# domerin0/rnn-speech

Measured on AMD Instinct MI355X. Metric: audio_frames_per_sec_train_3x512_lstm_ctc, higher is better.
Workload: dtype f32

## Files before the change

### include/amdspeech.h

```cpp
#ifndef AMDSPEECH_H
#define AMDSPEECH_H

#include <stddef.h>
#include <stdint.h>

#ifdef __cplusplus
extern "C" {
#endif

#define AMDSPEECH_OK 0
#define AMDSPEECH_EINVAL (-1)
#define AMDSPEECH_EHIP (-2)
#define AMDSPEECH_EUNSUPPORTED (-3)
#define AMDSPEECH_ETIMEOUT (-4)

int amdspeech_version(void);
const char* amdspeech_last_error(void);
int amdspeech_device_cu_count(void);

int amdspeech_linear_fwd(void* stream, const float* x, const float* w, const float* b,
                         float* y, int M, int K, int N);
int amdspeech_linear_bwd(void* stream, const float* x, const float* w, const float* dy,
                         float* dx, float* dw, float* db, int M, int K, int N);

// ... 107 lines not shown
                           const float* kernels, long kernel_stride, const float* biases, long bias_stride,
                           const int* lengths, const float* h0, const float* c0, const amdspeech_ctc_head* head);
int amdspeech_lstm_bwd_ctc(void* stream, const amdspeech_lstm_desc* d, void* ws,
                           const float* kernels, long kernel_stride, float* dkernels, float* dbiases, long bias_stride,
                           const int* lengths, const amdspeech_ctc_head* head);

int amdspeech_lstm_dropout_multipliers(void* stream, const amdspeech_lstm_desc* d, int which, int layer, float* out);

enum { AMDSPEECH_LSTM_PATH_FLOW = 0, AMDSPEECH_LSTM_PATH_BIG1 = 1, AMDSPEECH_LSTM_PATH_BIG = 2, AMDSPEECH_LSTM_PATH_HOIST = 3,
       AMDSPEECH_LSTM_PATH_DIAG = 4, AMDSPEECH_LSTM_PATH_DIAG_BF3 = 5 };
typedef struct amdspeech_lstm_plan_info {
    int fwd_path, bwd_path, nmt, kb, mv, wpx, uw, fwd_mt, pair, bf16p, bf16p_reserved, xw_parts, nfw, w_pieces, dz0_inkernel, flow2_q;
} amdspeech_lstm_plan_info;
int amdspeech_lstm_plan(const amdspeech_lstm_desc* d, int C, int U, amdspeech_lstm_plan_info* out);
int amdspeech_lstm_plan_xw_halves(const amdspeech_lstm_desc* d, int C, int U);

enum {
    AMDSPEECH_BIDIR_WS_Z0 = 0, AMDSPEECH_BIDIR_WS_YTOP_FW = 1, AMDSPEECH_BIDIR_WS_YTOP_BW = 2, AMDSPEECH_BIDIR_WS_DYTOP_FW = 3,
    AMDSPEECH_BIDIR_WS_DYTOP_BW = 4, AMDSPEECH_BIDIR_WS_DZ0 = 5, AMDSPEECH_BIDIR_WS_HFINAL = 6, AMDSPEECH_BIDIR_WS_CFINAL = 7
};
size_t amdspeech_lstm_bidir_workspace_bytes(const amdspeech_lstm_desc* d);
void* amdspeech_lstm_bidir_ws_ptr(const amdspeech_lstm_desc* d, void* ws, int which);
long amdspeech_lstm_bidir_layer_stride(const amdspeech_lstm_desc* d);
int amdspeech_lstm_bidir_path(const amdspeech_lstm_desc* d);
int amdspeech_lstm_bidir_fwd(void* stream, const amdspeech_lstm_desc* d, void* ws, const float* const* kernels,
                             const float* const* biases, const int* lengths, const float* h0, const float* c0);
int amdspeech_lstm_bidir_bwd(void* stream, const amdspeech_lstm_desc* d, void* ws, const float* const* kernels,
                             float* const* dkernels, float* const* dbiases, const int* lengths);
int amdspeech_lstm_bidir_status(const amdspeech_lstm_desc* d, void* ws);
int amdspeech_lstm_bidir_dropout_multipliers(void* stream, const amdspeech_lstm_desc* d, int dir, int which, int layer, float* out);
// ... 202 lines not shown
```

### rnn-speech_amd/csrc/lstm.hip

```cpp
#include "common.h"
#include "gemm_core.h"
#include "ctc_core.h"
#include <stdlib.h>
#include <string.h>
#include <type_traits>
#include <mutex>
#include <unordered_map>

namespace amdspeech {

#define FLOW_WEIGHTS_RESIDENT() __builtin_amdgcn_s_waitcnt(0x0F70)
static unsigned long long* dev_trace_ptr() {
#ifdef AMDSPEECH_DEVTRACE
    if (const char* e = dev_knob_str("AMDSPEECH_TRACE_PTR")) return reinterpret_cast<unsigned long long*>(strtoull(e, nullptr, 0));
#endif
    return nullptr;
}
#ifndef BIG_WEIGHTS_RESIDENT
#define BIG_WEIGHTS_RESIDENT 1
#endif

struct LstmLayout {
    size_t wp, wq, z, hs, cs, gates, dg, dztop, dz0, dc, xp0, xp, hp, dgp, sync, xph, hph, dxh, prec, pdown, xwp, bigring, wopack, bfs, total;
    size_t fwd_set = 0;
// ... 291 lines not shown
}

static bool use_big_fwd(const amdspeech_lstm_desc* d) {
    static const int env = runtime_switch("AMDSPEECH_BIG", 1);
    return env != 0 && !(d->flags & AMDSPEECH_LSTM_PER_DIAGONAL) && d->precision >= 0 && d->precision <= 2 && d->H == 1024 &&
           (d->B + 15) / 16 <= 4 && device_cus() == 256 &&
           (size_t)2 * ((d->B + 15) / 16 * 16) * d->H * 4 < (1ull << 32);
}

static bool use_flow(const amdspeech_lstm_desc* d) {
    static const int env = runtime_switch("AMDSPEECH_FLOW", 1);
    return env != 0 && !(d->flags & AMDSPEECH_LSTM_PER_DIAGONAL) && flow_shape_ok(d) && device_cus() == 256 && d->L * ((d->B + 15) / 16) <= 8;
}

template <bool CF>
static void (*flow_fwd_kernel(int kb, int pr, int mv, int mh))(FlowArgs) {
    switch (kb) {
        case 1: return lstm_fwd_flow2<1, 0, 0, CF>;
        case 2: return pr == 2 ? lstm_fwd_flow2<2, 2, 0, CF> : (pr == 1 ? lstm_fwd_flow2<2, 1, 0, CF> : lstm_fwd_flow2<2, 0, 0, CF>);
        case 3: return lstm_fwd_flow2<3, 0, 0, CF>;
        default:
            if (pr == 0 && mv == 1) return mh == 1 ? lstm_fwd_flow2<4, 0, 1, CF, 1> : lstm_fwd_flow2<4, 0, 1, CF>;
            return pr == 2 ? lstm_fwd_flow2<4, 2, 0, CF> : (pr == 1 ? lstm_fwd_flow2<4, 1, 0, CF> : lstm_fwd_flow2<4, 0, 0, CF>);
    }
}
template <bool CF>
static void (*flow_bwd_kernel(int kb, int pr))(FlowBwdArgs) {
    if (pr == 2) return kb == 2 ? lstm_bwd_flow2<2, 2, CF> : lstm_bwd_flow2<4, 2, CF>;
    if (pr == 1) return kb == 2 ? lstm_bwd_flow2<2, 1, CF> : lstm_bwd_flow2<4, 1, CF>;
    return kb == 1 ? lstm_bwd_flow2<1, 0, CF> : (kb == 2 ? lstm_bwd_flow2<2, 0, CF> : (kb == 3 ? lstm_bwd_flow2<3, 0, CF> : lstm_bwd_flow2<4, 0, CF>));
}
static int flow_fill_fwd_panels(hipStream_t s, const amdspeech_lstm_desc* d, float* ws, const LstmLayout& lo, int set) {
    const size_t bph = (size_t)(d->B + 15) / 16 * 16 * d->H;
    float* base = ws + (size_t)set * lo.fwd_set;
    AS_CHECK_HIP(hipMemsetD32Async(reinterpret_cast<hipDeviceptr_t>(base + lo.xph + (size_t)d->T * bph), (int)FLOW_SENTINEL,
                                   (size_t)d->L * d->T * bph, s));
    AS_CHECK_HIP(hipMemsetD32Async(reinterpret_cast<hipDeviceptr_t>(base + lo.hph), (int)FLOW_SENTINEL, (size_t)d->L * (d->T + 1) * bph, s));
// ... 140 lines not shown
    int xw_half;
    bool big_ring;
    bool bf16p_reserved;
    bool bf16p;
    Path fwd, bwd;
    bool pair;
    int uw;
    unsigned long long limit;
    void (*fwd_diag)(FwdArgs); int fwd_mt;
    void (*bwd_diag)(BwdArgs);
    void (*fwd_big)(BigFwdArgs); void (*bwd_big)(BigBwdArgs);
    void (*fwd_flow)(FlowArgs); void (*bwd_flow)(FlowBwdArgs);
    size_t fwd_lds, bwd_lds;
    int mv, wpx, wpw;
    int mh;
    int nfw;
    int dz0_inkernel;
    int w_pieces, w_t0, w_dz0;
    bool w_deal;
};

struct FlowGemmShare { int pieces, percent; bool set; };
static FlowGemmShare flow_gemm_share() {
    static const FlowGemmShare g = [] {
        FlowGemmShare r{8, 38, false};
        if (const char* e = dev_knob_str("AMDSPEECH_FLOW_GEMM")) {
            r.set = true;
            r.pieces = atoi(e);
            if (const char* q = strchr(e, ':')) r.percent = atoi(q + 1);
        }
// ... 24 lines not shown
    const Path diag = pr != 0 ? Path::diag_bf3 : Path::diag;
    p.fwd = flow ? Path::flow : big ? (p.pair && big1_env == 2 ? Path::big1 : Path::big) : diag;
    p.bwd = flow ? Path::flow : (p.pair && p.bf16p) ? Path::big1 : big ? Path::big
          : (pr == 0 && H >= 768 && p.nmt >= 2) ? Path::hoist : diag;
    p.uw = (flow || big) ? 16 : pick_uw(d);

    p.fwd_mt = p.nmt % 2 == 0 ? 2 : 1;
    if (pr != 0) p.fwd_diag = lstm_fwd_step_bf3<8>;
    else if (p.uw == 8) p.fwd_diag = p.fwd_mt == 2 ? lstm_fwd_step<8, 8, 8, false, 2> : lstm_fwd_step<8, 8, 8, false, 1>;
    else p.fwd_diag = p.fwd_mt == 2 ? lstm_fwd_step<4, 8, 8, false, 2> : lstm_fwd_step<4, 8, 8, false, 1>;
    p.bwd_diag = pr != 0 ? lstm_bwd_step_bf3<8> : lstm_bwd_step<8, 8, true>;
    p.fwd_big = pr == 2 ? lstm_fwd_big<2> : (pr == 1 ? lstm_fwd_big<1> : lstm_fwd_big<0>);
    p.bwd_big = pr == 2 ? lstm_bwd_big<2> : (pr == 1 ? lstm_bwd_big<1> : lstm_bwd_big<0>);
    if (!flow) return p;

    static const int workers_env = runtime_switch("AMDSPEECH_FLOW_FWD_WORKERS", 2);
    const int groups = L * p.nmt, spare = 8 - groups;
    p.wpw = 8;
    if (workers_env != 0 && p.xw_parts > 0)
        for (int waves = 4; waves <= 8 && p.mv == 0; waves += 4) {
            const int per = fwd_worker_wgs_per_xcd(d, waves);
            if (per <= 32 - FWD2_WORKER_RESERVE) { p.mv = 1; p.wpx = per; p.wpw = waves; }
        }
    p.mh = (workers_env != 1 && p.mv == 1 && p.wpw == 4 && p.xw_half > 0) ? 1 : 0;
    if (head != nullptr) p.nfw = ctc_head_nfw(d, head->C, head->U, p.wpx);
    const int kb = H / 128;
    p.fwd_flow = head != nullptr ? flow_fwd_kernel<true>(kb, pr, p.mv, p.mh) : flow_fwd_kernel<false>(kb, pr, p.mv, p.mh);
    p.bwd_flow = head != nullptr ? flow_bwd_kernel<true>(kb, pr) : flow_bwd_kernel<false>(kb, pr);
    p.fwd_lds = head != nullptr ? (size_t)2 * CF_FOLLOW_TEAM_FLOATS * sizeof(float) : 0;
    p.bwd_lds = ((size_t)2 * 1024 + 2 * 8 * 256 + (FLOW2_WINDOW ? 2 : 1) * 8 * kb * 256 + (size_t)(flow2_q(kb, pr) - 1) * 1024) * sizeof(float);
    const size_t lds_workers = (size_t)2 * 2 * 2 * BK * LDS_LD * sizeof(float);
    if (p.bwd_lds < lds_workers) p.bwd_lds = lds_workers;
    if (p.bwd_lds < (size_t)2 * CF_LEAD_TEAM_FLOATS * sizeof(float)) p.bwd_lds = (size_t)2 * CF_LEAD_TEAM_FLOATS * sizeof(float);

    const FlowGemmShare g = flow_gemm_share();
    const bool workers = g.pieces > 0 && g.percent > 0 && T >= 64 && groups < 8 && H % 128 == 0;
    const int share = g.set ? g.percent : (pr != 0 ? (head != nullptr ? g.percent / 2 - 1 : g.percent * 3 / 4) : g.percent);
    static const int dz0_in = runtime_switch("AMDSPEECH_FLOW_DZ0", 1);
    p.dz0_inkernel = dz0_in ? 1 : 0;
    p.w_dz0 = (p.dz0_inkernel || workers) ? 0 : 1;
    p.w_pieces = workers ? g.pieces : 0;
    static const int deal = runtime_switch("AMDSPEECH_FLOW_WORKER_DEAL", -1);
// ... 761 lines not shown
    const bool flow_bwd = p.bwd == Path::flow;
    static_assert((int)Path::flow == AMDSPEECH_LSTM_PATH_FLOW && (int)Path::big1 == AMDSPEECH_LSTM_PATH_BIG1 &&
                  (int)Path::big == AMDSPEECH_LSTM_PATH_BIG && (int)Path::hoist == AMDSPEECH_LSTM_PATH_HOIST &&
                  (int)Path::diag == AMDSPEECH_LSTM_PATH_DIAG && (int)Path::diag_bf3 == AMDSPEECH_LSTM_PATH_DIAG_BF3, "amdspeech.h");
    *out = amdspeech_lstm_plan_info{(int)p.fwd, (int)p.bwd, p.nmt, p.fwd == Path::flow ? d->H / 128 : 0, p.mv, p.wpx, p.uw, p.fwd_mt,
                                    p.pair ? 1 : 0, p.bf16p ? 1 : 0, p.bf16p_reserved ? 1 : 0, p.xw_parts, p.nfw, p.w_pieces,
                                    p.dz0_inkernel, flow_bwd ? flow2_q(d->H / 128, d->precision) : 0};
    return AMDSPEECH_OK;
}
extern "C" int amdspeech_lstm_plan_xw_halves(const amdspeech_lstm_desc* d, int C, int U) {
    if (check_desc(d) != AMDSPEECH_OK) return -1;
    amdspeech_ctc_head h{};
    h.C = C; h.U = U;
    const LstmPlan p = lstm_plan(d, C > 0 ? &h : nullptr);
    return 2 * p.mv + p.mh;
}
extern "C" int amdspeech_lstm_ctc_fusable(const amdspeech_lstm_desc* d, int C, int U) {
    if (check_desc(d) != AMDSPEECH_OK) return 0;
    amdspeech_ctc_head h{};
    h.C = C; h.U = U;
    return lstm_plan(d, &h).nfw > 0 ? 1 : 0;
}
static int check_head(const amdspeech_ctc_head* h, bool bwd) {
    AS_CHECK_ARG(h != nullptr, "lstm_*_ctc: null head");
    AS_CHECK_ARG(h->w_out && h->b_out && h->logits && h->dense_labels && h->loss && h->ctc_ws && (!bwd || h->dlogits),
                 "lstm_*_ctc: null pointer in the head");
    AS_CHECK_ARG(((uintptr_t)h->w_out % 16) == 0 && ((uintptr_t)h->ctc_ws % 256) == 0, "lstm_*_ctc: W_o must be 16-byte, the CTC workspace 256-byte aligned");
    return AMDSPEECH_OK;
}
extern "C" int amdspeech_lstm_fwd_ctc(void* stream, const amdspeech_lstm_desc* d, void* ws, const float* kernels,
// ... 384 lines not shown
```

### rnn-speech_amd/csrc/lstm_flow_fwd.h

```cpp

#ifndef FWD2_GATHER_AT
#define FWD2_GATHER_AT 1
#endif
#ifndef FWD2_WORKER_LAG
#define FWD2_WORKER_LAG 4
#endif

template <int KB, int MV, int MH, int NTW>
__device__ __forceinline__ void fwd_x_worker(const FlowArgs& a, const int role, const int lane, const unsigned long long t_begin) {
    constexpr int H = 128 * KB, NKBX = H / 16, NU = H / 16, NT = 4;
    constexpr bool HALF = NTW != NT;
    constexpr int J0 = NT - NTW;
    static_assert(NTW == 4 || (NTW == 2 && MH == 1), "x-product workers: full roles, or half roles of a launch that carries them");
    const int T = a.T, nmt = (a.B + 15) / 16;
    int r = __builtin_amdgcn_readfirstlane(role);
    const int part = HALF ? MV : r % MV;
    if (!HALF) r /= MV;
    const int ub = r % NU; r /= NU;
    const int mb = r % nmt;
    const int l = r / nmt;
    if (l >= a.L) return;
    const size_t bph = (size_t)nmt * 16 * H;
    float4 w[8][NTW];
    {
        const float* wp = a.wp + ((size_t)(l * NU + ub) * (2 * NKBX)) * (NT * 256) + lane * 4;
#pragma unroll
        for (int wv = 0; wv < 8; ++wv)
#pragma unroll
            for (int j = 0; j < NTW; ++j) w[wv][j] = *reinterpret_cast<const float4*>(wp + (size_t)((wv * KB + KB - 1 - part) * NT + J0 + j) * 256);
    }
    const float* xsrc = l == 0 ? a.xp0 : a.xph + (size_t)l * T * bph;
    const auto rx = __builtin_amdgcn_make_buffer_rsrc(const_cast<float*>(xsrc), 0, (unsigned)((size_t)T * bph * 4), 0x00020000);
    const size_t fs = (size_t)a.L * nmt * NU * (MV * 1024 + MH * 512);
    const auto ro = __builtin_amdgcn_make_buffer_rsrc(a.xwp, 0, (unsigned)((size_t)T * fs * 4), 0x00020000);
    const unsigned lane_off = (unsigned)((((size_t)mb * NKBX + (KB - 1 - part)) * 256 + lane * 4) * 4);
    const unsigned out_off = HALF ? (unsigned)(((size_t)a.L * nmt * NU * MV * 1024 + (((size_t)l * nmt + mb) * NU + ub) * 512 + lane * 4) * 4)
                                  : (unsigned)((((((size_t)l * nmt + mb) * NU + ub) * MV + part) * 1024 + lane * 4) * 4);
    const unsigned par = a.xw_par & 1u;
    bool dead = false;
    u32x4_f xa[8] = {}, xb[8] = {};
    auto load_l2 = [&](u32x4_f& dst, unsigned vo, unsigned so) { asm volatile("buffer_load_dwordx4 %0, %1, %2, %3 offen" : "+v"(dst) : "v"(vo), "s"(rx), "s"(so)); };
    auto load_mem = [&](u32x4_f& dst, unsigned vo, unsigned so) { asm volatile("buffer_load_dwordx4 %0, %1, %2, %3 offen sc1" : "+v"(dst) : "v"(vo), "s"(rx), "s"(so)); };
    auto issue = [&](auto bottom, u32x4_f (&buf)[8], int t) {
        const unsigned base = (unsigned)((size_t)(t < T ? t : T - 1) * bph * 4);
#pragma unroll
        for (int wv = 0; wv < 8; ++wv) {
            const unsigned vo = lane_off + (unsigned)(wv * KB * 1024);
            if (decltype(bottom)::value) load_l2(buf[wv], vo, base); else load_mem(buf[wv], vo, base);
        }
    };
    FLOW_WEIGHTS_RESIDENT();
    u32x4_f pr = (u32x4_f){0u, 0u, 0u, 0u};
    auto probe = [&](int t) {
        const int tp = t + FWD2_WORKER_LAG < T ? t + FWD2_WORKER_LAG : T - 1;
        load_mem(pr, lane_off, (unsigned)((size_t)tp * bph * 4));
    };
    auto landed12 = [&](u32x4_f (&buf)[8]) {
        asm volatile("s_waitcnt vmcnt(%9)" : "+v"(pr), "+v"(buf[0]), "+v"(buf[1]), "+v"(buf[2]), "+v"(buf[3]), "+v"(buf[4]), "+v"(buf[5]), "+v"(buf[6]), "+v"(buf[7]) : "n"(8 + NTW));
    };
    auto landed0 = [&](u32x4_f (&buf)[8]) {
        asm volatile("s_waitcnt vmcnt(0)" : "+v"(pr), "+v"(buf[0]), "+v"(buf[1]), "+v"(buf[2]), "+v"(buf[3]), "+v"(buf[4]), "+v"(buf[5]), "+v"(buf[6]), "+v"(buf[7]));
    };
    auto pending_any = [&](const u32x4_f (&buf)[8]) -> bool {
        unsigned bad = 0u;
#pragma unroll
        for (int wv = 0; wv < 8; ++wv) bad |= (unsigned)flow_pending(buf[wv]);
        return bad != 0u;
    };
#if defined(AMDSPEECH_DEVTRACE) && AMDSPEECH_DEVTRACE == 5
    const bool wtracing = a.trace != nullptr && l == a.trace_layer && ub == 3 && mb == 0 && part == 0 && lane == 0;
#define FXWSTAMP(i) do { if (wtracing && t >= 500 && t < 508) a.trace[128 + (t - 500) * 8 + (i)] = wall_clock64(); } while (0)
#else
#define FXWSTAMP(i) do { } while (0)
#endif
    auto work = [&](auto bottom, int t, u32x4_f (&buf)[8]) __attribute__((always_inline)) {
        FXWSTAMP(0);
        landed12(buf);
        FXWSTAMP(1);
        if (!decltype(bottom)::value) {
            if (__any(flow_pending(pr) || pending_any(buf)) && !dead) {
                while (true) {
                    if (wall_clock64() - t_begin > a.limit) { dead = true; if (lane == 0) atomicOr(a.err, 8u); break; }
                    __builtin_amdgcn_s_sleep(4);
                    probe(t);
                    issue(bottom, buf, t);
                    landed0(buf);
                    if (!__any(flow_pending(pr) || pending_any(buf))) break;
                }
            }
        }
        FXWSTAMP(2);
        probe(t + 1);
        f32x4 acc[NTW];
#pragma unroll
        for (int j = 0; j < NTW; ++j) acc[j] = (f32x4){0.f, 0.f, 0.f, 0.f};
#pragma unroll
        for (int wv = 0; wv < 8; ++wv)
#pragma unroll
            for (int j = 0; j < NTW; ++j) {
                acc[j] = __builtin_amdgcn_mfma_f32_16x16x4f32(__uint_as_float(buf[wv][0]), w[wv][j].x, acc[j], 0, 0, 0);
                acc[j] = __builtin_amdgcn_mfma_f32_16x16x4f32(__uint_as_float(buf[wv][1]), w[wv][j].y, acc[j], 0, 0, 0);
                acc[j] = __builtin_amdgcn_mfma_f32_16x16x4f32(__uint_as_float(buf[wv][2]), w[wv][j].z, acc[j], 0, 0, 0);
                acc[j] = __builtin_amdgcn_mfma_f32_16x16x4f32(__uint_as_float(buf[wv][3]), w[wv][j].w, acc[j], 0, 0, 0);
            }
        const unsigned fo = out_off + (unsigned)((size_t)t * fs * 4);
#pragma unroll
        for (int i = 0; i < NTW; ++i) {
            f32x4 v;
            if constexpr (HALF) v = (f32x4){acc[0][2 * i], acc[1][2 * i], acc[0][2 * i + 1], acc[1][2 * i + 1]};
            else v = (f32x4){acc[0][i], acc[1][i], acc[2][i], acc[3][i]};
            __builtin_amdgcn_raw_buffer_store_b128(flow_tag(v, par), ro, fo + (unsigned)(i * 1024), 0, 16);
        }
        __builtin_amdgcn_sched_barrier(0);
        FXWSTAMP(3);
        issue(bottom, buf, t + 2);
        FXWSTAMP(4);
    };
#undef FXWSTAMP
    auto run = [&](auto bottom) __attribute__((always_inline)) {
        probe(0);
        if (!decltype(bottom)::value) {
            landed0(xa);
            if (__any(flow_pending(pr)) && !dead) {
                while (true) {
                    if (wall_clock64() - t_begin > a.limit) { dead = true; if (lane == 0) atomicOr(a.err, 8u); break; }
                    __builtin_amdgcn_s_sleep(4);
                    probe(0);
                    landed0(xa);
                    if (!__any(flow_pending(pr))) break;
                }
            }
        }
        issue(bottom, xa, 0);
        landed0(xa);
        issue(bottom, xb, 1);
        for (int t = 0; t < T; t += 2) {
            work(bottom, t, xa);
            if (t + 1 < T) work(bottom, t + 1, xb);
        }
        landed0(xa);
        landed0(xb);
    };
    if (l == 0) run(std::true_type{}); else run(std::false_type{});
}

#define FLOW_G(T, p) ((T __attribute__((address_space(1)))*)(p))
template <typename Args>
__device__ __forceinline__ Args flow_args_again() {
    typedef unsigned args_u4 __attribute__((ext_vector_type(4)));
    typedef const args_u4 __attribute__((address_space(4))) * cptr;
    static_assert(sizeof(Args) % 16 == 0, "argument struct: a whole number of 16-byte pieces");
    unsigned long long p = (unsigned long long)__builtin_amdgcn_kernarg_segment_ptr();
    asm("" : "+s"(p));
    const cptr q = (cptr)p;
    args_u4 buf[sizeof(Args) / 16];
#pragma unroll
    for (unsigned i = 0; i < sizeof(Args) / 16; ++i) buf[i] = q[i];
    Args r;
    __builtin_memcpy(&r, buf, sizeof(Args));
    return r;
}
template <int H>
__device__ __forceinline__ void ctc_follower_call(const CtcFlow& c, int wg, int nwg) {
    extern __shared__ __attribute__((aligned(16))) float cf_lds[];
    if (c.B <= nwg * 2) ctc_follower<H, 1>(c, cf_lds, wg, nwg);
    else ctc_follower<H, 2>(c, cf_lds, wg, nwg);
}

template <int KB, int PR, int MV, bool CF = false, int MH = 0>
__global__ __launch_bounds__(512) void lstm_fwd_flow2(FlowArgs a_in) {
    constexpr bool BF3 = PR != 0;
    static_assert(MV >= 0 && MV < KB && (MV == 0 || PR == 0), "x-product workers: exact f32 only, and one K block of the x half stays");
    static_assert(MH == 0 || (MH == 1 && MV > 0 && KB - MV >= 2), "half roles: beside full roles, and one whole K block of the x half stays");
    constexpr int KX = KB - MV;
    constexpr int NTL = MH ? 2 : 4;
    constexpr int MVA = MV > 0 ? MV : 1;
    constexpr int UW = 16, NT = 4, H = 128 * KB, NKBX = H / 16, NW = 8;
    __shared__ __attribute__((aligned(16))) float red_[1][NW][256][NT];
    __shared__ __attribute__((aligned(16))) float outbox[2][8][256];
    __shared__ unsigned s_ticket;
    const int lane = threadIdx.x & 63, wave = __builtin_amdgcn_readfirstlane(threadIdx.x >> 6);
    unsigned xcc;
    asm volatile("s_getreg_b32 %0, hwreg(HW_REG_XCC_ID)" : "=s"(xcc));
    xcc &= 0xF;
    if (threadIdx.x == 0) s_ticket = atomicAdd(a_in.tickets + xcc, 1u);
    __syncthreads();
    const int grp = (int)xcc, ub = __builtin_amdgcn_readfirstlane((int)s_ticket);
    if (grp >= a_in.L * ((a_in.B + 15) / 16)) {
        const int first = a_in.L * ((a_in.B + 15) / 16);
        if (MV > 0 && ub < a_in.w_wpx && wave < a_in.w_wpw)
            fwd_x_worker<KB, MVA, MH, 4>(a_in, (((grp - first) * a_in.w_wpx + ub) * a_in.w_wpw + wave), lane, wall_clock64());
        else if (MH > 0 && ub < a_in.w_wpx) {
            if constexpr (MH > 0) fwd_x_worker<KB, MVA, MH, 2>(a_in, (((grp - first) * a_in.w_wpx + ub) * 4 + wave - 4), lane, wall_clock64());
        }
        else if (CF && a_in.cf_on && ub >= a_in.w_wpx && ub < a_in.w_wpx + a_in.cf_nfw) {
            if constexpr (CF) ctc_follower_call<H>(a_in.cf, (grp - first) * a_in.cf_nfw + (ub - a_in.w_wpx), (8 - first) * a_in.cf_nfw);
        }
        return;
    }
    const FlowArgs a = CF ? flow_args_again<FlowArgs>() : a_in;
    const int T = a.T, B = a.B;
    const int nmt = (B + 15) / 16;
    if (ub >= H / UW) return;
    const int l = grp / nmt, mb = grp % nmt;
    const size_t bph = (size_t)nmt * 16 * H;
    const unsigned long long t_begin = wall_clock64();
    const unsigned long long c_begin = __builtin_readcyclecounter();

    float4 wx[KX][NT], wh[KB][NT];
    {
        const float __attribute__((address_space(1)))* wp = FLOW_G(const float, a.wp) + ((size_t)(l * (H / UW) + ub) * (2 * NKBX)) * (NT * 256) + lane * 4;
#pragma unroll
        for (int kb = 0; kb < KB; ++kb)
#pragma unroll
            for (int j = 0; j < NT; ++j) {
                if (kb < KX && (kb < KX - 1 || j < NTL)) { const f32x4 v = *(const f32x4 __attribute__((address_space(1)))*)(wp + (size_t)((wave * KB + kb) * NT + j) * 256); wx[kb][j] = make_float4(v[0], v[1], v[2], v[3]); }
                { const f32x4 v = *(const f32x4 __attribute__((address_space(1)))*)(wp + (size_t)((NKBX + wave * KB + kb) * NT + j) * 256); wh[kb][j] = make_float4(v[0], v[1], v[2], v[3]); }
            }
    }
    constexpr int KP = BF3 ? KB / 2 : 1;
    u32x4_f wxh[KP][NT], wxl[KP][NT], whh[KP][NT], whl[KP][NT];
    if constexpr (BF3) {
#pragma unroll
        for (int jb = 0; jb < KB / 2; ++jb)
#pragma unroll
            for (int j = 0; j < NT; ++j) {
                const float xx[8] = {wx[2 * jb][j].x, wx[2 * jb][j].y, wx[2 * jb][j].z, wx[2 * jb][j].w,
                                     wx[2 * jb + 1][j].x, wx[2 * jb + 1][j].y, wx[2 * jb + 1][j].z, wx[2 * jb + 1][j].w};
                flow_bf3_split(xx, wxh[jb][j], wxl[jb][j]);
                const float xh[8] = {wh[2 * jb][j].x, wh[2 * jb][j].y, wh[2 * jb][j].z, wh[2 * jb][j].w,
                                     wh[2 * jb + 1][j].x, wh[2 * jb + 1][j].y, wh[2 * jb + 1][j].z, wh[2 * jb + 1][j].w};
// ... 144 lines not shown
#pragma unroll
        for (int j = 0; j < NJ; ++j) acc[j] = __builtin_amdgcn_mfma_f32_16x16x4f32(__uint_as_float(v[2]), w[j].z, acc[j], 0, 0, 0);
#pragma unroll
        for (int j = 0; j < NJ; ++j) acc[j] = __builtin_amdgcn_mfma_f32_16x16x4f32(__uint_as_float(v[3]), w[j].w, acc[j], 0, 0, 0);
        __builtin_amdgcn_sched_barrier(0);
#else
#pragma unroll
        for (int j = 0; j < NJ; ++j) {
            acc[j] = __builtin_amdgcn_mfma_f32_16x16x4f32(__uint_as_float(v[0]), w[j].x, acc[j], 0, 0, 0);
            acc[j] = __builtin_amdgcn_mfma_f32_16x16x4f32(__uint_as_float(v[1]), w[j].y, acc[j], 0, 0, 0);
            acc[j] = __builtin_amdgcn_mfma_f32_16x16x4f32(__uint_as_float(v[2]), w[j].z, acc[j], 0, 0, 0);
            acc[j] = __builtin_amdgcn_mfma_f32_16x16x4f32(__uint_as_float(v[3]), w[j].w, acc[j], 0, 0, 0);
        }
#endif
    };
    auto half_product = [&](const auto& v, const auto& w, const u32x4_f (&wh_)[KP][NT], const u32x4_f (&wl_)[KP][NT],
                            auto between, auto last_tiles) __attribute__((always_inline)) {
        constexpr int NB = (int)(sizeof(v) / sizeof(v[0]));
        if constexpr (BF3) {
#pragma unroll
            for (int jb = 0; jb < KB / 2; ++jb) {
                between(2 * jb);
                between(2 * jb + 1);
                const float x[8] = {__uint_as_float(v[2 * jb][0]), __uint_as_float(v[2 * jb][1]), __uint_as_float(v[2 * jb][2]),
                                    __uint_as_float(v[2 * jb][3]), __uint_as_float(v[2 * jb + 1][0]), __uint_as_float(v[2 * jb + 1][1]),
                                    __uint_as_float(v[2 * jb + 1][2]), __uint_as_float(v[2 * jb + 1][3])};
                u32x4_f ah, al;
                flow_bf3_split(x, ah, al);
#pragma unroll
                for (int j = 0; j < NT; ++j) acc[j] = flow_bf_mma<PR>(acc[j], ah, al, wh_[jb][j], wl_[jb][j]);
            }
        } else {
#pragma unroll
            for (int kb = 0; kb < NB; ++kb) {
                between(kb);
                if (kb == NB - 1) mma_block(v[kb], w[kb], last_tiles);
                else mma_block(v[kb], w[kb], std::integral_constant<int, NT>{});
            }
        }
    };
    auto fsig = [](float x) __attribute__((always_inline)) { return __builtin_amdgcn_rcpf(1.0f + __builtin_amdgcn_exp2f(-1.4426950408889634f * x)); };
    auto ftanh = [](float x) __attribute__((always_inline)) {
        const float x2 = x * x;
        const float small = x * (1.0f + x2 * (-0.33333334f + x2 * (0.13333334f - 0.053968254f * x2)));
        const float big = 1.0f - 2.0f * __builtin_amdgcn_rcpf(1.0f + __builtin_amdgcn_exp2f(2.8853900817779268f * x));
        return fabsf(x) < 0.25f ? small : big;
    };
    auto stores = [&](int t) __attribute__((always_inline)) {
        const int sl = threadIdx.x - 256;
        const float (&ob)[8][256] = outbox[t & 1];
        const float zv = ob[6][sl] * zmult(a.drop, l + 1, (uint32_t)((size_t)t * B * H + e));
// ... 27 lines not shown
        const float cv = live ? cn : c_prev;
        const float zv = live ? hn : 0.0f;
        __hip_atomic_store(FLOW_G(float, a.hph) + ((size_t)l * (T + 1) + t + 1) * bph + po, hval, __ATOMIC_RELAXED, __HIP_MEMORY_SCOPE_WORKGROUP);
        const int sl = threadIdx.x;
        float (&ob)[8][256] = outbox[t & 1];
        ob[0][sl] = gi; ob[1][sl] = gj; ob[2][sl] = gf; ob[3][sl] = go;
        ob[4][sl] = cv; ob[5][sl] = hval; ob[6][sl] = zv; ob[7][sl] = c_prev;
        c_prev = cv; h_prev = hval;
    };
    auto x_half = [&](auto xpol, int t, u32x4_f (&xnext)[KX], bool gather_h) __attribute__((always_inline)) {
#pragma unroll
        for (int j = 0; j < NT; ++j) acc[j] = (f32x4){0.f, 0.f, 0.f, 0.f};
        if (t + 1 < T) {
            if (decltype(xpol)::value != 2 && !(ASM && FWD2_EARLY_XCHECK)) settle(Remote{}, xnext, rx, (unsigned)((size_t)(t + 1) * bph * 4));
            half_product(xnext, wx, wxh, wxl, [&](int kb) {
                if (gather_h && kb == (FWD2_GATHER_AT < KX ? FWD2_GATHER_AT : KX - 1)) {
                    __builtin_amdgcn_sched_barrier(0);
                    issue(Local{}, hv, rh, (unsigned)((size_t)(t + 1) * bph * 4));
                    __builtin_amdgcn_sched_barrier(0);
                }
            }, std::integral_constant<int, NTL>{});
        }
    };
#ifndef FWD2_ISSUE_AT_TOP
#define FWD2_ISSUE_AT_TOP 0
#endif
    constexpr bool TOP = ASM && FWD2_ISSUE_AT_TOP != 0;
    auto step = [&](auto xpol, int t, u32x4_f (&xnext)[KX], u32x4_f (&xfree)[KX], u32x4_f (&wcur)[MVA], u32x4_f (&wfree)[MVA],
                    u32x2_f& hcur, u32x2_f& hfree) __attribute__((always_inline)) {
        F2STAMP(0);
        if constexpr (TOP) {
// ... 96 lines not shown
```

### rnn-speech_amd/lib.py

```python
import ctypes as C
import os

HERE = os.path.dirname(os.path.abspath(__file__))
LIB_PATH = os.environ.get("AMDSPEECH_LIB") or os.path.join(HERE, "libamdspeech.so")


class AmdSpeechError(RuntimeError):
    pass


class DataflowTimeout(AmdSpeechError):
    """amdspeech_lstm_status returned AMDSPEECH_ETIMEOUT: a whole-sequence launch gave up waiting.  The mini-batch's results are
    invalid; it can be repeated on the launch-per-diagonal kernels.  Any OTHER error of that call is a device fault."""


ETIMEOUT = -4
ECALLBACK = -100


class LstmDesc(C.Structure):
    _fields_ = [("T", C.c_int), ("B", C.c_int), ("H", C.c_int), ("L", C.c_int),
                ("keep_in", C.c_float), ("keep_out", C.c_float), ("seed", C.c_uint64),
                ("precision", C.c_int), ("flags", C.c_int)]

# ... 117 lines not shown
    "amdspeech_lstm_fwd": (_I, [_P, C.POINTER(LstmDesc), _P, _P, _L, _P, _L, _P, _P, _P]),
    "amdspeech_lstm_status": (_I, [C.POINTER(LstmDesc), _P]),
    "amdspeech_lstm_workspace_release": (_I, [_P, _P]),
    "amdspeech_lstm_beside_forward": (_I, [_P, _P]),
    "amdspeech_lstm_beside_tail": (_I, [_P, _P]),
    "amdspeech_lstm_bwd": (_I, [_P, C.POINTER(LstmDesc), _P, _P, _L, _P, _P, _L, _P]),
    "amdspeech_lstm_ctc_fusable": (_I, [C.POINTER(LstmDesc), _I, _I]),
    "amdspeech_lstm_pair_fusable": (_I, [C.POINTER(LstmDesc)]),
    "amdspeech_lstm_fwd_pair": (_I, [_P, C.POINTER(LstmDesc), _P, _P, _P, C.POINTER(LstmDesc), _P, _P, _P, _L, _L, _P, _P, _P]),
    "amdspeech_lstm_bwd_pair": (_I, [_P, C.POINTER(LstmDesc), _P, _P, _P, _P, C.POINTER(LstmDesc), _P, _P, _P, _P, _L, _L, _P]),
    "amdspeech_lstm_fwd_ctc": (_I, [_P, C.POINTER(LstmDesc), _P, _P, _L, _P, _L, _P, _P, _P, C.POINTER(CtcHead)]),
    "amdspeech_lstm_bwd_ctc": (_I, [_P, C.POINTER(LstmDesc), _P, _P, _L, _P, _P, _L, _P, C.POINTER(CtcHead)]),
    "amdspeech_lstm_dropout_multipliers": (_I, [_P, C.POINTER(LstmDesc), _I, _I, _P]),
    "amdspeech_lstm_plan": (_I, [C.POINTER(LstmDesc), _I, _I, C.POINTER(LstmPlanInfo)]),
    "amdspeech_lstm_plan_xw_halves": (_I, [C.POINTER(LstmDesc), _I, _I]),
    "amdspeech_lstm_bidir_workspace_bytes": (_SZ, [C.POINTER(LstmDesc)]),
    "amdspeech_lstm_bidir_ws_ptr": (_P, [C.POINTER(LstmDesc), _P, _I]),
    "amdspeech_lstm_bidir_layer_stride": (_L, [C.POINTER(LstmDesc)]),
    "amdspeech_lstm_bidir_path": (_I, [C.POINTER(LstmDesc)]),
    "amdspeech_lstm_bidir_fwd": (_I, [_P, C.POINTER(LstmDesc), _P, _P, _P, _P, _P, _P]),
    "amdspeech_lstm_bidir_bwd": (_I, [_P, C.POINTER(LstmDesc), _P, _P, _P, _P, _P]),
    "amdspeech_lstm_bidir_status": (_I, [C.POINTER(LstmDesc), _P]),
    "amdspeech_lstm_bidir_dropout_multipliers": (_I, [_P, C.POINTER(LstmDesc), _I, _I, _I, _P]),
    "amdspeech_ctc_workspace_bytes": (_SZ, [_I, _I, _I, _I]),
    "amdspeech_ctc_plan": (_I, [_I, _I, _I, _I, C.POINTER(CtcPlanInfo)]),
    "amdspeech_ctc_loss_fwd_bwd": (_I, [_P, _P, _P, _P, _I, _I, _I, _I, _P, _P, _P]),
    "amdspeech_ctc_loss_fwd_bwd_staged": (_I, [_P, _P, _P, _P, _I, _I, _I, _I, _P, _P, _P, _I]),
    "amdspeech_ctc_align_workspace_bytes": (_SZ, [_I, _I, _I, _I]),
    "amdspeech_ctc_align_plan": (_I, [_I, _I, _I, _I, C.POINTER(CtcPlanInfo)]),
    "amdspeech_ctc_align": (_I, [_P, _P, _P, _P, _I, _I, _I, _I, _P, _P, _P, _P, _P, _P]),
# ... 98 lines not shown
```

### rnn-speech_amd/ops.py

```python
import ctypes as C
import os

import torch

from . import lib as _l

MODE_MFCC, MODE_FBANK = 0, 1


def _stream():
    return C.c_void_p(torch.cuda.current_stream().cuda_stream)


def _p(t):
    return C.c_void_p(t.data_ptr()) if t is not None else C.c_void_p(0)


def _chk_f32(*ts):
    for t in ts:
        if t is None:
            continue
        if not (t.is_cuda and t.dtype == torch.float32 and t.is_contiguous()):
            raise ValueError("expected a contiguous float32 device tensor, got %s %s" % (t.dtype, t.device))

# ... 343 lines not shown
                    _l.LSTM_PER_DIAGONAL if per_diagonal else 0)
    info = _l.LstmPlanInfo()
    _l.check(ws.lib.amdspeech_lstm_plan(C.byref(d), c_u[0], c_u[1], C.byref(info)), "lstm_plan")
    out = _plan_dict(info)
    out["fwd_path"], out["bwd_path"] = _l.LSTM_PATHS[out["fwd_path"]], _l.LSTM_PATHS[out["bwd_path"]]
    return out


def lstm_plan_xw_halves(ws, head=None, per_diagonal=False):
    c_u = (0, 0) if head is None else ((head.c.C, head.c.U) if isinstance(head, CtcHead) else (int(head[0]), int(head[1])))
    d = _l.LstmDesc(ws.desc.T, ws.desc.B, ws.desc.H, ws.desc.L, ws.desc.keep_in, ws.desc.keep_out, ws.desc.seed, ws.desc.precision,
                    _l.LSTM_PER_DIAGONAL if per_diagonal else 0)
    n = int(ws.lib.amdspeech_lstm_plan_xw_halves(C.byref(d), c_u[0], c_u[1]))
    if n < 0:
        raise ValueError("lstm_plan_xw_halves: bad descriptor")
    return n


def lstm_fwd(ws, kernels, kernel_stride, biases, bias_stride, lengths, h0=None, c0=None, training=False, per_diagonal=False, head=None):
    _chk_i32(lengths)
    _chk_f32(h0, c0)
    root, key = ws._root, (ws.T, int(ws.desc.precision))
    if per_diagonal:
        root._armed, training = None, False
    armed = _ARM and root._armed is not None and root._armed["fwd"] == key
    root._armed = None
    inject, root._inject_timeout = getattr(root, "_inject_timeout", 0), 0
    ws.desc.flags = ((_l.LSTM_ARMED if armed else 0) | (_l.LSTM_ARM_NEXT if (training and _ARM) else 0) |
                     (_l.LSTM_SAME_WS if (root._fwd_seen and _ARM) else 0) | (_l.LSTM_PER_DIAGONAL if per_diagonal else 0) |
                     (_l.LSTM_INJECT_TIMEOUT if inject else 0))
# ... 837 lines not shown
```

Before: 2.731 million.

## Offload extra x-product k-steps from recurrent waves to half-role x workers

Adds an extended mode for the half-role x-product workers in the flow forward kernel. Each of these workers now also computes 2 or 3 extra k-steps from the K block below its own, using extra dwordx2/x3 buffer loads and weights held in registers. The recurrent waves skip those k-steps in a trimmed MFMA block, which shortens the per-timestep critical path. The default worker setting moves from 2 to 3 so the mode is on by default, and a plan query is exported to report it. The cost is more registers and loads per worker, a different gather point, and more complex sentinel and wait-count handling.

```diff
diff --git a/include/amdspeech.h b/include/amdspeech.h
--- a/include/amdspeech.h
+++ b/include/amdspeech.h
@@ -145,6 +145,7 @@
 } amdspeech_lstm_plan_info;
 int amdspeech_lstm_plan(const amdspeech_lstm_desc* d, int C, int U, amdspeech_lstm_plan_info* out);
 int amdspeech_lstm_plan_xw_halves(const amdspeech_lstm_desc* d, int C, int U);
+int amdspeech_lstm_plan_xw_ksteps(const amdspeech_lstm_desc* d, int C, int U);
 
 enum {
     AMDSPEECH_BIDIR_WS_Z0 = 0, AMDSPEECH_BIDIR_WS_YTOP_FW = 1, AMDSPEECH_BIDIR_WS_YTOP_BW = 2, AMDSPEECH_BIDIR_WS_DYTOP_FW = 3,
diff --git a/rnn-speech_amd/csrc/lstm.hip b/rnn-speech_amd/csrc/lstm.hip
--- a/rnn-speech_amd/csrc/lstm.hip
+++ b/rnn-speech_amd/csrc/lstm.hip
@@ -329,13 +329,14 @@
 }
 
 template <bool CF>
-static void (*flow_fwd_kernel(int kb, int pr, int mv, int mh))(FlowArgs) {
+static void (*flow_fwd_kernel(int kb, int pr, int mv, int mh, int me))(FlowArgs) {
     switch (kb) {
         case 1: return lstm_fwd_flow2<1, 0, 0, CF>;
         case 2: return pr == 2 ? lstm_fwd_flow2<2, 2, 0, CF> : (pr == 1 ? lstm_fwd_flow2<2, 1, 0, CF> : lstm_fwd_flow2<2, 0, 0, CF>);
         case 3: return lstm_fwd_flow2<3, 0, 0, CF>;
         default:
-            if (pr == 0 && mv == 1) return mh == 1 ? lstm_fwd_flow2<4, 0, 1, CF, 1> : lstm_fwd_flow2<4, 0, 1, CF>;
+            if (pr == 0 && mv == 1 && mh == 1) return me > 0 ? lstm_fwd_flow2<4, 0, 1, CF, 1, FWD2_HALF_KSTEPS> : lstm_fwd_flow2<4, 0, 1, CF, 1>;
+            if (pr == 0 && mv == 1) return lstm_fwd_flow2<4, 0, 1, CF>;
             return pr == 2 ? lstm_fwd_flow2<4, 2, 0, CF> : (pr == 1 ? lstm_fwd_flow2<4, 1, 0, CF> : lstm_fwd_flow2<4, 0, 0, CF>);
     }
 }
@@ -506,6 +507,7 @@
     size_t fwd_lds, bwd_lds;
     int mv, wpx, wpw;
     int mh;
+    int me;
     int nfw;
     int dz0_inkernel;
     int w_pieces, w_t0, w_dz0;
@@ -560,7 +562,7 @@
     p.bwd_big = pr == 2 ? lstm_bwd_big<2> : (pr == 1 ? lstm_bwd_big<1> : lstm_bwd_big<0>);
     if (!flow) return p;
 
-    static const int workers_env = runtime_switch("AMDSPEECH_FLOW_FWD_WORKERS", 2);
+    static const int workers_env = runtime_switch("AMDSPEECH_FLOW_FWD_WORKERS", 3);
     const int groups = L * p.nmt, spare = 8 - groups;
     p.wpw = 8;
     if (workers_env != 0 && p.xw_parts > 0)
@@ -569,9 +571,10 @@
             if (per <= 32 - FWD2_WORKER_RESERVE) { p.mv = 1; p.wpx = per; p.wpw = waves; }
         }
     p.mh = (workers_env != 1 && p.mv == 1 && p.wpw == 4 && p.xw_half > 0) ? 1 : 0;
+    p.me = (p.mh == 1 && workers_env != 2) ? FWD2_HALF_KSTEPS : 0;
     if (head != nullptr) p.nfw = ctc_head_nfw(d, head->C, head->U, p.wpx);
     const int kb = H / 128;
-    p.fwd_flow = head != nullptr ? flow_fwd_kernel<true>(kb, pr, p.mv, p.mh) : flow_fwd_kernel<false>(kb, pr, p.mv, p.mh);
+    p.fwd_flow = head != nullptr ? flow_fwd_kernel<true>(kb, pr, p.mv, p.mh, p.me) : flow_fwd_kernel<false>(kb, pr, p.mv, p.mh, p.me);
     p.bwd_flow = head != nullptr ? flow_bwd_kernel<true>(kb, pr) : flow_bwd_kernel<false>(kb, pr);
     p.fwd_lds = head != nullptr ? (size_t)2 * CF_FOLLOW_TEAM_FLOATS * sizeof(float) : 0;
     p.bwd_lds = ((size_t)2 * 1024 + 2 * 8 * 256 + (FLOW2_WINDOW ? 2 : 1) * 8 * kb * 256 + (size_t)(flow2_q(kb, pr) - 1) * 1024) * sizeof(float);
@@ -1363,6 +1366,13 @@
     h.C = C; h.U = U;
     const LstmPlan p = lstm_plan(d, C > 0 ? &h : nullptr);
     return 2 * p.mv + p.mh;
+}
+extern "C" int amdspeech_lstm_plan_xw_ksteps(const amdspeech_lstm_desc* d, int C, int U) {
+    if (check_desc(d) != AMDSPEECH_OK) return -1;
+    amdspeech_ctc_head h{};
+    h.C = C; h.U = U;
+    const LstmPlan p = lstm_plan(d, C > 0 ? &h : nullptr);
+    return p.me;
 }
 extern "C" int amdspeech_lstm_ctc_fusable(const amdspeech_lstm_desc* d, int C, int U) {
     if (check_desc(d) != AMDSPEECH_OK) return 0;
diff --git a/rnn-speech_amd/csrc/lstm_flow_fwd.h b/rnn-speech_amd/csrc/lstm_flow_fwd.h
--- a/rnn-speech_amd/csrc/lstm_flow_fwd.h
+++ b/rnn-speech_amd/csrc/lstm_flow_fwd.h
@@ -2,16 +2,27 @@
 #ifndef FWD2_GATHER_AT
 #define FWD2_GATHER_AT 1
 #endif
+#ifndef FWD2_GATHER_AT_EXT
+#define FWD2_GATHER_AT_EXT 0
+#endif
 #ifndef FWD2_WORKER_LAG
 #define FWD2_WORKER_LAG 4
 #endif
+#ifndef FWD2_HALF_KSTEPS
+#define FWD2_HALF_KSTEPS 2
+#endif
 
-template <int KB, int MV, int MH, int NTW>
+template <int KB, int MV, int MH, int NTW, int ME = 0>
 __device__ __forceinline__ void fwd_x_worker(const FlowArgs& a, const int role, const int lane, const unsigned long long t_begin) {
     constexpr int H = 128 * KB, NKBX = H / 16, NU = H / 16, NT = 4;
     constexpr bool HALF = NTW != NT;
     constexpr int J0 = NT - NTW;
     static_assert(NTW == 4 || (NTW == 2 && MH == 1), "x-product workers: full roles, or half roles of a launch that carries them");
+    static_assert(ME == 0 || (NTW == 2 && (ME == 2 || ME == 3) && KB - 2 - MV >= 0), "extended half roles: 2 or 3 k-steps of the block below the half role's");
+    constexpr bool EXT = ME > 0;
+    constexpr int MEA = EXT ? ME : 2;
+    constexpr int NLD = 8 + (EXT ? 8 : 0);
+    typedef unsigned xe_t __attribute__((ext_vector_type(MEA)));
     const int T = a.T, nmt = (a.B + 15) / 16;
     int r = __builtin_amdgcn_readfirstlane(role);
     const int part = HALF ? MV : r % MV;
@@ -29,6 +40,16 @@
 #pragma unroll
             for (int j = 0; j < NTW; ++j) w[wv][j] = *reinterpret_cast<const float4*>(wp + (size_t)((wv * KB + KB - 1 - part) * NT + J0 + j) * 256);
     }
+    float we[8][2][MEA];
+    if constexpr (EXT) {
+        const float* wp = a.wp + ((size_t)(l * NU + ub) * (2 * NKBX)) * (NT * 256) + lane * 4 + (4 - ME);
+#pragma unroll
+        for (int wv = 0; wv < 8; ++wv)
+#pragma unroll
+            for (int j = 0; j < 2; ++j)
+#pragma unroll
+                for (int m = 0; m < ME; ++m) we[wv][j][m] = wp[(size_t)((wv * KB + KB - 2 - MV) * NT + J0 + j) * 256 + m];
+    }
     const float* xsrc = l == 0 ? a.xp0 : a.xph + (size_t)l * T * bph;
     const auto rx = __builtin_amdgcn_make_buffer_rsrc(const_cast<float*>(xsrc), 0, (unsigned)((size_t)T * bph * 4), 0x00020000);
     const size_t fs = (size_t)a.L * nmt * NU * (MV * 1024 + MH * 512);
@@ -39,32 +60,66 @@
     const unsigned par = a.xw_par & 1u;
     bool dead = false;
     u32x4_f xa[8] = {}, xb[8] = {};
-    auto load_l2 = [&](u32x4_f& dst, unsigned vo, unsigned so) { asm volatile("buffer_load_dwordx4 %0, %1, %2, %3 offen" : "+v"(dst) : "v"(vo), "s"(rx), "s"(so)); };
-    auto load_mem = [&](u32x4_f& dst, unsigned vo, unsigned so) { asm volatile("buffer_load_dwordx4 %0, %1, %2, %3 offen sc1" : "+v"(dst) : "v"(vo), "s"(rx), "s"(so)); };
-    auto issue = [&](auto bottom, u32x4_f (&buf)[8], int t) {
+    xe_t ea[8] = {}, eb[8] = {};
+    constexpr int MOFF = EXT ? 1024 : 0, EOFF = (4 - MEA) * 4;
+    const unsigned lane_base = lane_off - (unsigned)MOFF;
+    auto load_l2 = [&](u32x4_f& dst, unsigned vo, unsigned so) { asm volatile("buffer_load_dwordx4 %0, %1, %2, %3 offen offset:%4" : "+v"(dst) : "v"(vo), "s"(rx), "s"(so), "n"(MOFF)); };
+    auto load_mem = [&](u32x4_f& dst, unsigned vo, unsigned so) { asm volatile("buffer_load_dwordx4 %0, %1, %2, %3 offen offset:%4 sc1" : "+v"(dst) : "v"(vo), "s"(rx), "s"(so), "n"(MOFF)); };
+    auto ext_l2 = [&](xe_t& dst, unsigned vo, unsigned so) {
+        if constexpr (ME == 3) asm volatile("buffer_load_dwordx3 %0, %1, %2, %3 offen offset:%4" : "+v"(dst) : "v"(vo), "s"(rx), "s"(so), "n"(EOFF));
+        else asm volatile("buffer_load_dwordx2 %0, %1, %2, %3 offen offset:%4" : "+v"(dst) : "v"(vo), "s"(rx), "s"(so), "n"(EOFF));
+    };
+    auto ext_mem = [&](xe_t& dst, unsigned vo, unsigned so) {
+        if constexpr (ME == 3) asm volatile("buffer_load_dwordx3 %0, %1, %2, %3 offen offset:%4 sc1" : "+v"(dst) : "v"(vo), "s"(rx), "s"(so), "n"(EOFF));
+        else asm volatile("buffer_load_dwordx2 %0, %1, %2, %3 offen offset:%4 sc1" : "+v"(dst) : "v"(vo), "s"(rx), "s"(so), "n"(EOFF));
+    };
+    auto issue = [&](auto bottom, u32x4_f (&buf)[8], xe_t (&ebuf)[8], int t) {
         const unsigned base = (unsigned)((size_t)(t < T ? t : T - 1) * bph * 4);
 #pragma unroll
         for (int wv = 0; wv < 8; ++wv) {
-            const unsigned vo = lane_off + (unsigned)(wv * KB * 1024);
-            if (decltype(bottom)::value) load_l2(buf[wv], vo, base); else load_mem(buf[wv], vo, base);
+            const unsigned vo = EXT ? lane_base : lane_base + (unsigned)(wv * KB * 1024);
+            const unsigned so = EXT ? base + (unsigned)(wv * KB * 1024) : base;
+            if (decltype(bottom)::value) load_l2(buf[wv], vo, so); else load_mem(buf[wv], vo, so);
+        }
+        if constexpr (EXT) {
+#pragma unroll
+            for (int wv = 0; wv < 8; ++wv) {
+                const unsigned so = base + (unsigned)(wv * KB * 1024);
+                if (decltype(bottom)::value) ext_l2(ebuf[wv], lane_base, so); else ext_mem(ebuf[wv], lane_base, so);
+            }
         }
     };
     FLOW_WEIGHTS_RESIDENT();
     u32x4_f pr = (u32x4_f){0u, 0u, 0u, 0u};
     auto probe = [&](int t) {
         const int tp = t + FWD2_WORKER_LAG < T ? t + FWD2_WORKER_LAG : T - 1;
-        load_mem(pr, lane_off, (unsigned)((size_t)tp * bph * 4));
-    };
-    auto landed12 = [&](u32x4_f (&buf)[8]) {
-        asm volatile("s_waitcnt vmcnt(%9)" : "+v"(pr), "+v"(buf[0]), "+v"(buf[1]), "+v"(buf[2]), "+v"(buf[3]), "+v"(buf[4]), "+v"(buf[5]), "+v"(buf[6]), "+v"(buf[7]) : "n"(8 + NTW));
-    };
-    auto landed0 = [&](u32x4_f (&buf)[8]) {
-        asm volatile("s_waitcnt vmcnt(0)" : "+v"(pr), "+v"(buf[0]), "+v"(buf[1]), "+v"(buf[2]), "+v"(buf[3]), "+v"(buf[4]), "+v"(buf[5]), "+v"(buf[6]), "+v"(buf[7]));
-    };
-    auto pending_any = [&](const u32x4_f (&buf)[8]) -> bool {
+        load_mem(pr, lane_base, (unsigned)((size_t)tp * bph * 4));
+    };
+    constexpr int FRAME_INFLIGHT = NLD + NTW;
+    auto landed12 = [&](u32x4_f (&buf)[8], xe_t (&ebuf)[8]) {
+        if constexpr (EXT)
+            asm volatile("s_waitcnt vmcnt(%17)" : "+v"(pr), "+v"(buf[0]), "+v"(buf[1]), "+v"(buf[2]), "+v"(buf[3]), "+v"(buf[4]), "+v"(buf[5]), "+v"(buf[6]), "+v"(buf[7]),
+                         "+v"(ebuf[0]), "+v"(ebuf[1]), "+v"(ebuf[2]), "+v"(ebuf[3]), "+v"(ebuf[4]), "+v"(ebuf[5]), "+v"(ebuf[6]), "+v"(ebuf[7]) : "n"(FRAME_INFLIGHT));
+        else
+            asm volatile("s_waitcnt vmcnt(%9)" : "+v"(pr), "+v"(buf[0]), "+v"(buf[1]), "+v"(buf[2]), "+v"(buf[3]), "+v"(buf[4]), "+v"(buf[5]), "+v"(buf[6]), "+v"(buf[7]) : "n"(FRAME_INFLIGHT));
+    };
+    auto landed0 = [&](u32x4_f (&buf)[8], xe_t (&ebuf)[8]) {
+        if constexpr (EXT)
+            asm volatile("s_waitcnt vmcnt(0)" : "+v"(pr), "+v"(buf[0]), "+v"(buf[1]), "+v"(buf[2]), "+v"(buf[3]), "+v"(buf[4]), "+v"(buf[5]), "+v"(buf[6]), "+v"(buf[7]),
+                         "+v"(ebuf[0]), "+v"(ebuf[1]), "+v"(ebuf[2]), "+v"(ebuf[3]), "+v"(ebuf[4]), "+v"(ebuf[5]), "+v"(ebuf[6]), "+v"(ebuf[7]));
+        else
+            asm volatile("s_waitcnt vmcnt(0)" : "+v"(pr), "+v"(buf[0]), "+v"(buf[1]), "+v"(buf[2]), "+v"(buf[3]), "+v"(buf[4]), "+v"(buf[5]), "+v"(buf[6]), "+v"(buf[7]));
+    };
+    auto pending_any = [&](const u32x4_f (&buf)[8], const xe_t (&ebuf)[8]) -> bool {
         unsigned bad = 0u;
 #pragma unroll
         for (int wv = 0; wv < 8; ++wv) bad |= (unsigned)flow_pending(buf[wv]);
+        if constexpr (EXT) {
+#pragma unroll
+            for (int wv = 0; wv < 8; ++wv)
+#pragma unroll
+                for (int m = 0; m < ME; ++m) bad |= (unsigned)(ebuf[wv][m] == FLOW_SENTINEL);
+        }
         return bad != 0u;
     };
 #if defined(AMDSPEECH_DEVTRACE) && AMDSPEECH_DEVTRACE == 5
@@ -73,19 +128,19 @@
 #else
 #define FXWSTAMP(i) do { } while (0)
 #endif
-    auto work = [&](auto bottom, int t, u32x4_f (&buf)[8]) __attribute__((always_inline)) {
+    auto work = [&](auto bottom, int t, u32x4_f (&buf)[8], xe_t (&ebuf)[8]) __attribute__((always_inline)) {
         FXWSTAMP(0);
-        landed12(buf);
+        landed12(buf, ebuf);
         FXWSTAMP(1);
         if (!decltype(bottom)::value) {
-            if (__any(flow_pending(pr) || pending_any(buf)) && !dead) {
+            if (__any(flow_pending(pr) || pending_any(buf, ebuf)) && !dead) {
                 while (true) {
                     if (wall_clock64() - t_begin > a.limit) { dead = true; if (lane == 0) atomicOr(a.err, 8u); break; }
                     __builtin_amdgcn_s_sleep(4);
                     probe(t);
-                    issue(bottom, buf, t);
-                    landed0(buf);
-                    if (!__any(flow_pending(pr) || pending_any(buf))) break;
+                    issue(bottom, buf, ebuf, t);
+                    landed0(buf, ebuf);
+                    if (!__any(flow_pending(pr) || pending_any(buf, ebuf))) break;
                 }
             }
         }
@@ -103,6 +158,15 @@
                 acc[j] = __builtin_amdgcn_mfma_f32_16x16x4f32(__uint_as_float(buf[wv][2]), w[wv][j].z, acc[j], 0, 0, 0);
                 acc[j] = __builtin_amdgcn_mfma_f32_16x16x4f32(__uint_as_float(buf[wv][3]), w[wv][j].w, acc[j], 0, 0, 0);
             }
+        if constexpr (EXT) {
+#pragma unroll
+            for (int wv = 0; wv < 8; ++wv)
+#pragma unroll
+                for (int j = 0; j < 2; ++j)
+#pragma unroll
+                    for (int m = 0; m < ME; ++m)
+                        acc[j] = __builtin_amdgcn_mfma_f32_16x16x4f32(__uint_as_float(ebuf[wv][m]), we[wv][j][m], acc[j], 0, 0, 0);
+        }
         const unsigned fo = out_off + (unsigned)((size_t)t * fs * 4);
 #pragma unroll
         for (int i = 0; i < NTW; ++i) {
@@ -113,33 +177,33 @@
         }
         __builtin_amdgcn_sched_barrier(0);
         FXWSTAMP(3);
-        issue(bottom, buf, t + 2);
+        issue(bottom, buf, ebuf, t + 2);
         FXWSTAMP(4);
     };
 #undef FXWSTAMP
     auto run = [&](auto bottom) __attribute__((always_inline)) {
         probe(0);
         if (!decltype(bottom)::value) {
-            landed0(xa);
+            landed0(xa, ea);
             if (__any(flow_pending(pr)) && !dead) {
                 while (true) {
                     if (wall_clock64() - t_begin > a.limit) { dead = true; if (lane == 0) atomicOr(a.err, 8u); break; }
                     __builtin_amdgcn_s_sleep(4);
                     probe(0);
-                    landed0(xa);
+                    landed0(xa, ea);
                     if (!__any(flow_pending(pr))) break;
                 }
             }
         }
-        issue(bottom, xa, 0);
-        landed0(xa);
-        issue(bottom, xb, 1);
+        issue(bottom, xa, ea, 0);
+        landed0(xa, ea);
+        issue(bottom, xb, eb, 1);
         for (int t = 0; t < T; t += 2) {
-            work(bottom, t, xa);
-            if (t + 1 < T) work(bottom, t + 1, xb);
-        }
-        landed0(xa);
-        landed0(xb);
+            work(bottom, t, xa, ea);
+            if (t + 1 < T) work(bottom, t + 1, xb, eb);
+        }
+        landed0(xa, ea);
+        landed0(xb, eb);
     };
     if (l == 0) run(std::true_type{}); else run(std::false_type{});
 }
@@ -167,11 +231,12 @@
     else ctc_follower<H, 2>(c, cf_lds, wg, nwg);
 }
 
-template <int KB, int PR, int MV, bool CF = false, int MH = 0>
+template <int KB, int PR, int MV, bool CF = false, int MH = 0, int ME = 0>
 __global__ __launch_bounds__(512) void lstm_fwd_flow2(FlowArgs a_in) {
     constexpr bool BF3 = PR != 0;
     static_assert(MV >= 0 && MV < KB && (MV == 0 || PR == 0), "x-product workers: exact f32 only, and one K block of the x half stays");
     static_assert(MH == 0 || (MH == 1 && MV > 0 && KB - MV >= 2), "half roles: beside full roles, and one whole K block of the x half stays");
+    static_assert(ME == 0 || (MH == 1 && (ME == 2 || ME == 3)), "extended half roles: 2 or 3 k-steps, in a launch with half roles");
     constexpr int KX = KB - MV;
     constexpr int NTL = MH ? 2 : 4;
     constexpr int MVA = MV > 0 ? MV : 1;
@@ -189,9 +254,9 @@
     if (grp >= a_in.L * ((a_in.B + 15) / 16)) {
         const int first = a_in.L * ((a_in.B + 15) / 16);
         if (MV > 0 && ub < a_in.w_wpx && wave < a_in.w_wpw)
-            fwd_x_worker<KB, MVA, MH, 4>(a_in, (((grp - first) * a_in.w_wpx + ub) * a_in.w_wpw + wave), lane, wall_clock64());
+            fwd_x_worker<KB, MVA, MH, 4, 0>(a_in, (((grp - first) * a_in.w_wpx + ub) * a_in.w_wpw + wave), lane, wall_clock64());
         else if (MH > 0 && ub < a_in.w_wpx) {
-            if constexpr (MH > 0) fwd_x_worker<KB, MVA, MH, 2>(a_in, (((grp - first) * a_in.w_wpx + ub) * 4 + wave - 4), lane, wall_clock64());
+            if constexpr (MH > 0) fwd_x_worker<KB, MVA, MH, 2, ME>(a_in, (((grp - first) * a_in.w_wpx + ub) * 4 + wave - 4), lane, wall_clock64());
         }
         else if (CF && a_in.cf_on && ub >= a_in.w_wpx && ub < a_in.w_wpx + a_in.cf_nfw) {
             if constexpr (CF) ctc_follower_call<H>(a_in.cf, (grp - first) * a_in.cf_nfw + (ub - a_in.w_wpx), (8 - first) * a_in.cf_nfw);
@@ -214,7 +279,11 @@
         for (int kb = 0; kb < KB; ++kb)
 #pragma unroll
             for (int j = 0; j < NT; ++j) {
-                if (kb < KX && (kb < KX - 1 || j < NTL)) { const f32x4 v = *(const f32x4 __attribute__((address_space(1)))*)(wp + (size_t)((wave * KB + kb) * NT + j) * 256); wx[kb][j] = make_float4(v[0], v[1], v[2], v[3]); }
+                if (ME > 0 && kb == KX - 2 && j >= 2) {
+                    const float __attribute__((address_space(1)))* q = wp + (size_t)((wave * KB + kb) * NT + j) * 256;
+                    wx[kb][j] = make_float4(q[0], ME < 3 ? q[1] : 0.0f, 0.0f, 0.0f);
+                }
+                else if (kb < KX && (kb < KX - 1 || j < NTL)) { const f32x4 v = *(const f32x4 __attribute__((address_space(1)))*)(wp + (size_t)((wave * KB + kb) * NT + j) * 256); wx[kb][j] = make_float4(v[0], v[1], v[2], v[3]); }
                 { const f32x4 v = *(const f32x4 __attribute__((address_space(1)))*)(wp + (size_t)((NKBX + wave * KB + kb) * NT + j) * 256); wh[kb][j] = make_float4(v[0], v[1], v[2], v[3]); }
             }
     }
@@ -389,6 +458,15 @@
         }
 #endif
     };
+    auto mma_block_cut = [&](const u32x4_f& v, const float4 (&w)[NT]) __attribute__((always_inline)) {
+#pragma unroll
+        for (int j = 0; j < NT; ++j) {
+            acc[j] = __builtin_amdgcn_mfma_f32_16x16x4f32(__uint_as_float(v[0]), w[j].x, acc[j], 0, 0, 0);
+            if (j < 2 || ME < 3) acc[j] = __builtin_amdgcn_mfma_f32_16x16x4f32(__uint_as_float(v[1]), w[j].y, acc[j], 0, 0, 0);
+            if (j < 2) acc[j] = __builtin_amdgcn_mfma_f32_16x16x4f32(__uint_as_float(v[2]), w[j].z, acc[j], 0, 0, 0);
+            if (j < 2) acc[j] = __builtin_amdgcn_mfma_f32_16x16x4f32(__uint_as_float(v[3]), w[j].w, acc[j], 0, 0, 0);
+        }
+    };
     auto half_product = [&](const auto& v, const auto& w, const u32x4_f (&wh_)[KP][NT], const u32x4_f (&wl_)[KP][NT],
                             auto between, auto last_tiles) __attribute__((always_inline)) {
         constexpr int NB = (int)(sizeof(v) / sizeof(v[0]));
@@ -410,6 +488,7 @@
             for (int kb = 0; kb < NB; ++kb) {
                 between(kb);
                 if (kb == NB - 1) mma_block(v[kb], w[kb], last_tiles);
+                else if (ME > 0 && decltype(last_tiles)::value < NT && kb == NB - 2) mma_block_cut(v[kb], w[kb]);
                 else mma_block(v[kb], w[kb], std::integral_constant<int, NT>{});
             }
         }
@@ -467,7 +546,8 @@
         if (t + 1 < T) {
             if (decltype(xpol)::value != 2 && !(ASM && FWD2_EARLY_XCHECK)) settle(Remote{}, xnext, rx, (unsigned)((size_t)(t + 1) * bph * 4));
             half_product(xnext, wx, wxh, wxl, [&](int kb) {
-                if (gather_h && kb == (FWD2_GATHER_AT < KX ? FWD2_GATHER_AT : KX - 1)) {
+                constexpr int GAT = ME > 0 ? FWD2_GATHER_AT_EXT : FWD2_GATHER_AT;
+                if (gather_h && kb == (GAT < KX ? GAT : KX - 1)) {
                     __builtin_amdgcn_sched_barrier(0);
                     issue(Local{}, hv, rh, (unsigned)((size_t)(t + 1) * bph * 4));
                     __builtin_amdgcn_sched_barrier(0);
diff --git a/rnn-speech_amd/lib.py b/rnn-speech_amd/lib.py
--- a/rnn-speech_amd/lib.py
+++ b/rnn-speech_amd/lib.py
@@ -155,6 +155,7 @@
     "amdspeech_lstm_dropout_multipliers": (_I, [_P, C.POINTER(LstmDesc), _I, _I, _P]),
     "amdspeech_lstm_plan": (_I, [C.POINTER(LstmDesc), _I, _I, C.POINTER(LstmPlanInfo)]),
     "amdspeech_lstm_plan_xw_halves": (_I, [C.POINTER(LstmDesc), _I, _I]),
+    "amdspeech_lstm_plan_xw_ksteps": (_I, [C.POINTER(LstmDesc), _I, _I]),
     "amdspeech_lstm_bidir_workspace_bytes": (_SZ, [C.POINTER(LstmDesc)]),
     "amdspeech_lstm_bidir_ws_ptr": (_P, [C.POINTER(LstmDesc), _P, _I]),
     "amdspeech_lstm_bidir_layer_stride": (_L, [C.POINTER(LstmDesc)]),
diff --git a/rnn-speech_amd/ops.py b/rnn-speech_amd/ops.py
--- a/rnn-speech_amd/ops.py
+++ b/rnn-speech_amd/ops.py
@@ -381,6 +381,16 @@
     n = int(ws.lib.amdspeech_lstm_plan_xw_halves(C.byref(d), c_u[0], c_u[1]))
     if n < 0:
         raise ValueError("lstm_plan_xw_halves: bad descriptor")
+    return n
+
+
+def lstm_plan_xw_ksteps(ws, head=None, per_diagonal=False):
+    c_u = (0, 0) if head is None else ((head.c.C, head.c.U) if isinstance(head, CtcHead) else (int(head[0]), int(head[1])))
+    d = _l.LstmDesc(ws.desc.T, ws.desc.B, ws.desc.H, ws.desc.L, ws.desc.keep_in, ws.desc.keep_out, ws.desc.seed, ws.desc.precision,
+                    _l.LSTM_PER_DIAGONAL if per_diagonal else 0)
+    n = int(ws.lib.amdspeech_lstm_plan_xw_ksteps(C.byref(d), c_u[0], c_u[1]))
+    if n < 0:
+        raise ValueError("lstm_plan_xw_ksteps: bad descriptor")
     return n
 
 
```

After: 2.762 million, median of 6. 1.01x the previous value.
